# svenstaro/bvh

Hardware: NVIDIA H100
Metric: traversal_Mrays_per_s (higher is better)
Workload: dtype f32

## Files before the change

### bvh_b200/csrc/traverse.cu

```cuda
#include "internal.h"
#include "csr.cuh"
#include "queries.cuh"
#include <cstdlib>
#include <cstring>
#include <algorithm>
#include <chrono>

namespace bvhb200 {

static inline uint32_t pick_slots(bvhgpu_ctx* ctx, uint32_t nrays) {
    if (ctx->traverse_slots >= 0) return (uint32_t)std::min<int64_t>(ctx->traverse_slots, 64);
    uint64_t budget_words = 1ull << 30;
    if (ctx->slot_budget_words == 0) {
        size_t free_b = 0, total_b = 0;
        ctx->slot_budget_words = cudaMemGetInfo(&free_b, &total_b) == cudaSuccess ? std::max<uint64_t>((uint64_t)free_b / 16, 1) : budget_words;
    }
    budget_words = std::min<uint64_t>(budget_words, ctx->slot_budget_words);
    const uint64_t k = budget_words / std::max<uint32_t>(nrays, 1u);
    if (k < 4) return (uint32_t)k;
    uint32_t p = 4;
    while (p * 2 <= k && p < 64) p *= 2;
    return p;
}

template <class T> static inline const typename Traits<T>::DAabb* walk_aabbs(const Tree<T>* tree) { return tree->dims == 2 && tree->d_aabb_trav ? tree->d_aabb_trav : tree->d_aabb; }

constexpr int SCAN_ITEMS = 8;
constexpr int SCAN_THREADS = 256;
constexpr int SCAN_TILE = SCAN_ITEMS * SCAN_THREADS;
static_assert(SCAN_THREADS == CSR_SCAN_THREADS && SCAN_TILE == CSR_SCAN_TILE, "scan geometry declared in internal.h");

template <class T> __device__ __forceinline__ T tmin2(T a, T b);
template <> __device__ __forceinline__ float tmin2(float a, float b) { return fminf(a, b); }
template <> __device__ __forceinline__ double tmin2(double a, double b) { return fmin(a, b); }
template <class T> __device__ __forceinline__ T tmax2(T a, T b);
template <> __device__ __forceinline__ float tmax2(float a, float b) { return fmaxf(a, b); }
template <> __device__ __forceinline__ double tmax2(double a, double b) { return fmax(a, b); }

template <class T>
__device__ __forceinline__ bool slab_hit(const T o[3], const T inv[3], const T mn[3], const T mx[3]) {
    const T l0 = mul_rn(sub_rn(mn[0], o[0]), inv[0]), r0 = mul_rn(sub_rn(mx[0], o[0]), inv[0]);
    const T l1 = mul_rn(sub_rn(mn[1], o[1]), inv[1]), r1 = mul_rn(sub_rn(mx[1], o[1]), inv[1]);
    const T l2 = mul_rn(sub_rn(mn[2], o[2]), inv[2]), r2 = mul_rn(sub_rn(mx[2], o[2]), inv[2]);
    const bool nan = (l0 != l0) | (r0 != r0) | (l1 != l1) | (r1 != r1) | (l2 != l2) | (r2 != r2);
    const T tmin = tmax2(tmax2(tmin2(l0, r0), tmin2(l1, r1)), tmin2(l2, r2));
    const T tmax = tmin2(tmin2(tmax2(l0, r0), tmax2(l1, r1)), tmax2(l2, r2));
    const T lo = tmin > T(0) ? tmin : T(0);
    return !nan && tmax >= lo;
}
__device__ __forceinline__ float fmin_nan(float a, float b) { float r; asm("min.NaN.f32 %0, %1, %2;" : "=f"(r) : "f"(a), "f"(b)); return r; }
__device__ __forceinline__ float fmax_nan(float a, float b) { float r; asm("max.NaN.f32 %0, %1, %2;" : "=f"(r) : "f"(a), "f"(b)); return r; }
template <>
__device__ __forceinline__ bool slab_hit<float>(const float o[3], const float inv[3], const float mn[3], const float mx[3]) {
    const float l0 = mul_rn(sub_rn(mn[0], o[0]), inv[0]), r0 = mul_rn(sub_rn(mx[0], o[0]), inv[0]);
    const float l1 = mul_rn(sub_rn(mn[1], o[1]), inv[1]), r1 = mul_rn(sub_rn(mx[1], o[1]), inv[1]);
    const float l2 = mul_rn(sub_rn(mn[2], o[2]), inv[2]), r2 = mul_rn(sub_rn(mx[2], o[2]), inv[2]);
    const float tmin = fmax_nan(fmax_nan(fmin_nan(l0, r0), fmin_nan(l1, r1)), fmin_nan(l2, r2));
    const float tmax = fmin_nan(fmin_nan(fmax_nan(l0, r0), fmax_nan(l1, r1)), fmax_nan(l2, r2));
    const float lo = tmin > 0.f ? tmin : 0.f;
    return tmax >= lo;
}

template <class T, bool FLAT, class Emit>
__device__ __forceinline__ uint32_t walk(const typename Traits<T>::TNode* __restrict__ trec, uint32_t n_rec,
                                         const typename Traits<T>::DAabb* __restrict__ aabb,
                                         const T o[3], const T inv[3], Emit emit) {
    uint32_t i = 0, visits = 0;
    while (i < n_rec) {
        T mn[3], mx[3];
        uint32_t skip, shape;
        fetch(trec + i, mn, mx, skip, shape);
        ++visits;
        if (slab_hit(o, inv, mn, mx)) {
            if (shape != BVH_INVALID) {
                bool report = true;
                if (FLAT) {
                    T smn[3], smx[3];
                    load_aabb(aabb + shape, smn, smx);
                    report = slab_hit(o, inv, smn, smx);
                }
                if (report) emit(shape);
            }
            i = i + 1;
        } else {
            i = skip;
        }
    }
    return visits;
}

template <class T> struct RaySrc { const T* base; uint32_t fmt; };
constexpr uint32_t RAYS_FULL = 0, RAYS_OD = 1;
template <class T, bool L2>
__device__ __forceinline__ void load_ray(const RaySrc<T>& src, size_t r, T o[3], T inv[3]) {
    if (src.fmt == RAYS_FULL) {
        const T* p = src.base + 9 * r;
#pragma unroll
        for (int k = 0; k < 3; ++k) { o[k] = L2 ? __ldcg(p + k) : __ldg(p + k); inv[k] = L2 ? __ldcg(p + 6 + k) : __ldg(p + 6 + k); }
    } else {
        const T* p = src.base + 6 * r;
#pragma unroll
        for (int k = 0; k < 3; ++k) { o[k] = L2 ? __ldcg(p + k) : __ldg(p + k); inv[k] = div_rn(T(1), L2 ? __ldcg(p + 3 + k) : __ldg(p + 3 + k)); }
    }
}

template <class T>
__global__ void __launch_bounds__(256) coherence_probe_kernel(RaySrc<T> rays, uint32_t nrays, uint32_t* flag) {
    __shared__ float acc[8];
    float sum = 0.f;
    const uint32_t samples = 1024, stride = nrays > 2 * samples ? nrays / samples : 1;
    const uint32_t rstride = rays.fmt == RAYS_FULL ? 9u : 6u;
    uint32_t n = 0;
    for (uint32_t k = threadIdx.x; k < samples; k += 256) {
        const uint32_t i = k * stride;
        if (i + 1 >= nrays) break;
        const T* a = rays.base + (size_t)rstride * i + 3;
        const T* b = rays.base + (size_t)rstride * (i + 1) + 3;
        sum += (float)(a[0] * b[0] + a[1] * b[1] + a[2] * b[2]);
        ++n;
    }
    for (int o = 16; o > 0; o >>= 1) { sum += __shfl_xor_sync(0xffffffffu, sum, o); n += __shfl_xor_sync(0xffffffffu, n, o); }
    __shared__ uint32_t cnt[8];
    if (lane_id() == 0) { acc[threadIdx.x >> 5] = sum; cnt[threadIdx.x >> 5] = n; }
    __syncthreads();
    if (threadIdx.x == 0) {
        float s = 0.f; uint32_t c = 0;
        for (int w = 0; w < 8; ++w) { s += acc[w]; c += cnt[w]; }
        *flag = (c > 0 && s / (float)c > 0.9f) ? 1u : 0u;
    }
}

template <class T, bool FLAT>
__global__ void __launch_bounds__(256) walk_count_kernel(const typename Traits<T>::TNode* __restrict__ trec, uint32_t n_rec,
                                                         const typename Traits<T>::DAabb* __restrict__ aabb,
                                                         RaySrc<T> rays, uint32_t nrays,
                                                         uint32_t first, uint32_t count,
                                                         uint32_t* __restrict__ counts, uint32_t* __restrict__ slots, uint32_t K,
                                                         unsigned long long* __restrict__ visit_total, const uint32_t* __restrict__ gate, uint32_t run_if) {
    if (gate && *gate != run_if) return;
    const uint32_t r = first + blockIdx.x * blockDim.x + threadIdx.x;
    uint32_t visits = 0;
    if (r < first + count) {
        T o[3], inv[3];
        load_ray<T, false>(rays, r, o, inv);
        uint32_t cnt = 0;
        visits = walk<T, FLAT>(trec, n_rec, aabb, o, inv, [&](uint32_t shape) {
            if (cnt < K) slots[(size_t)cnt * nrays + r] = shape;
            ++cnt;
        });
        counts[r] = cnt;
    }
    visits = __reduce_add_sync(0xffffffffu, visits);
    if (lane_id() == 0 && visits) atomicAdd(visit_total, (unsigned long long)visits);
}

template <class T, bool FLAT, bool STREAM>
__global__ void __launch_bounds__(256) walk_persistent_kernel(const typename Traits<T>::TNode* __restrict__ trec, uint32_t n_rec,
                                                              const typename Traits<T>::DAabb* __restrict__ aabb,
                                                              RaySrc<T> rays, uint32_t nrays,
                                                              uint32_t* __restrict__ ticket, const uint32_t* ready,
                                                              uint32_t* __restrict__ counts, uint32_t* __restrict__ slots, uint32_t K,
                                                              unsigned long long* __restrict__ visit_total, const uint32_t* __restrict__ gate, uint32_t run_if,
                                                              uint32_t* err, unsigned long long timeout_ns) {
    if (gate && *gate != run_if) return;
    constexpr uint32_t NONE = 0xFFFFFFFFu;
    constexpr int REFILL = 8;
    const uint32_t FULL = 0xffffffffu;
    const uint32_t lane = lane_id(), lt = lanemask_lt();
    uint32_t r = NONE, i = 0, cnt = 0, visits = 0;
    bool loaded = false;
    T o[3] = {T(0), T(0), T(0)}, inv[3] = {T(0), T(0), T(0)};
    bool exhausted = false;
    for (;;) {
        const uint32_t need = __ballot_sync(FULL, r == NONE);
        if (need && !exhausted) {
            uint32_t base = 0;
            if (lane == 0) base = atomicAdd(ticket, (uint32_t)__popc(need));
            base = __shfl_sync(FULL, base, 0);
            if (base >= nrays) exhausted = true;
            const uint32_t mine = base + __popc(need & lt);
            if (r == NONE && mine < nrays) {
                r = mine; i = 0; cnt = 0;
                if (STREAM) loaded = false;
                else load_ray<T, false>(rays, mine, o, inv);
            }
        }
        if (STREAM) {
            const uint32_t pend = __ballot_sync(FULL, r != NONE && !loaded);
            if (pend) {
                const bool any_active = __ballot_sync(FULL, r != NONE && loaded) != 0u;
                const uint32_t lowest = __reduce_min_sync(FULL, (r != NONE && !loaded) ? r : NONE);
                uint32_t rd = 0, ok = 1;
                if (lane == 0) {
                    rd = *(volatile const uint32_t*)ready;
                    if (!any_active && rd <= lowest) {
                        uint32_t ns = 100;
                        const unsigned long long t0 = global_timer_ns();
                        while (rd <= lowest) {
                            if (*(volatile const uint32_t*)err != 0u) { ok = 0; break; }
                            if (global_timer_ns() - t0 > timeout_ns) { ok = 0; atomicExch(err, (uint32_t)BVHGPU_ERR_TIMEOUT); break; }
                            __nanosleep(ns);
                            if (ns < 2000) ns <<= 1;
                            rd = *(volatile const uint32_t*)ready;
                        }
                    }
                }
                rd = __shfl_sync(FULL, rd, 0);
                ok = __shfl_sync(FULL, ok, 0);
                if (!ok) {
                    exhausted = true;
                    if (r != NONE && !loaded) r = NONE;
                } else if (__ballot_sync(FULL, r != NONE && !loaded && r < rd)) {
                    __threadfence();
                    if (r != NONE && !loaded && r < rd) { load_ray<T, true>(rays, r, o, inv); loaded = true; }
                }
            }
        }
        if (__ballot_sync(FULL, r != NONE) == 0) break;
        uint32_t rounds = 0;
        for (;;) {
            if (r != NONE && (!STREAM || loaded)) {
                T mn[3], mx[3];
                uint32_t skip, shape;
                fetch(trec + i, mn, mx, skip, shape);
                ++visits;
                if (slab_hit(o, inv, mn, mx)) {
                    if (shape != BVH_INVALID) {
                        bool report = true;
                        if (FLAT) {
                            T smn[3], smx[3];
                            load_aabb(aabb + shape, smn, smx);
                            report = slab_hit(o, inv, smn, smx);
                        }
                        if (report) { if (cnt < K) slots[(size_t)cnt * nrays + r] = shape; ++cnt; }
                    }
                    i = i + 1;
                } else {
                    i = skip;
                }
                if (i >= n_rec) { counts[r] = cnt; r = NONE; }
            }
            const uint32_t idle_mask = __ballot_sync(FULL, r == NONE);
            const int idle = __popc(idle_mask);
            if (idle == 32 || (idle >= REFILL && !exhausted)) break;
            if (STREAM) {
                const uint32_t pend = __ballot_sync(FULL, r != NONE && !loaded);
                if (pend && (((++rounds) & 15u) == 0u || (pend | idle_mask) == FULL)) break;
            }
        }
    }
    visits = __reduce_add_sync(FULL, visits);
    if (lane == 0 && visits) atomicAdd(visit_total, (unsigned long long)visits);
}

template <bool FLAT, bool STREAM, int VPC>
__global__ void __launch_bounds__(1024, 1) walk_top_kernel(const TNodeF* __restrict__ trec, const DAabbF* __restrict__ aabb,
                                                           uint32_t n_rec, const float4* __restrict__ top,
                                                           RaySrc<float> rays, uint32_t nrays, uint32_t* __restrict__ ticket, const uint32_t* ready,
                                                           uint32_t* __restrict__ counts, uint32_t* __restrict__ slots, uint32_t K,
                                                           unsigned long long* __restrict__ visit_total, const uint32_t* __restrict__ gate, uint32_t run_if,
                                                           uint32_t* err, unsigned long long timeout_ns, int refill) {
    extern __shared__ float4 s_top[];
    if (gate && *gate != run_if) return;
    const uint32_t n_top = reinterpret_cast<const uint32_t*>(top)[0];
    for (uint32_t k = threadIdx.x; k < 2 * n_top; k += blockDim.x) s_top[k] = top[2 + k];
    __syncthreads();
    uint32_t s_lo, s_hi;
    asm volatile("mov.u32 %0, %1;" : "=r"(s_lo) : "r"((uint32_t)__cvta_generic_to_shared(s_top)));
    asm volatile("mov.u32 %0, %1;" : "=r"(s_hi) : "r"(s_lo + 16u * n_top));
    constexpr uint32_t NONE = 0xFFFFFFFFu;
    const uint32_t FULL = 0xffffffffu;
    const uint32_t lane = lane_id(), lt = lanemask_lt();
    uint32_t r = NONE, j = NONE, g = 0, gend = 0, cnt = 0, visits = 0;
    bool loaded = false;
    float o[3] = {0.f, 0.f, 0.f}, inv[3] = {0.f, 0.f, 0.f};
    float4 a = make_float4(0.f, 0.f, 0.f, 0.f), b = a;
    bool exhausted = false;
    for (;;) {
        const uint32_t need = __ballot_sync(FULL, r == NONE);
        if (need && !exhausted) {
            uint32_t base = 0;
            if (lane == 0) base = atomicAdd(ticket, (uint32_t)__popc(need));
            base = __shfl_sync(FULL, base, 0);
            if (base >= nrays) exhausted = true;
            const uint32_t mine = base + __popc(need & lt);
            if (r == NONE && mine < nrays) {
                r = mine; cnt = 0; g = 0;
                if (STREAM) { loaded = false; j = NONE; gend = 0; }
                else { j = 0; gend = n_top ? 0u : n_rec; load_ray<float, false>(rays, mine, o, inv); }
            }
        }
        if (STREAM) {
            const uint32_t pend = __ballot_sync(FULL, r != NONE && !loaded);
            if (pend) {
                const bool any_active = __ballot_sync(FULL, r != NONE && loaded) != 0u;
                const uint32_t lowest = __reduce_min_sync(FULL, (r != NONE && !loaded) ? r : NONE);
                uint32_t rd = 0, ok = 1;
                if (lane == 0) {
                    rd = *(volatile const uint32_t*)ready;
                    if (!any_active && rd <= lowest) {
                        uint32_t ns = 100;
                        const unsigned long long t0 = global_timer_ns();
                        while (rd <= lowest) {
                            if (*(volatile const uint32_t*)err != 0u) { ok = 0; break; }
                            if (global_timer_ns() - t0 > timeout_ns) { ok = 0; atomicExch(err, (uint32_t)BVHGPU_ERR_TIMEOUT); break; }
                            __nanosleep(ns);
                            if (ns < 2000) ns <<= 1;
                            rd = *(volatile const uint32_t*)ready;
                        }
                    }
                }
                rd = __shfl_sync(FULL, rd, 0);
                ok = __shfl_sync(FULL, ok, 0);
                if (!ok) {
                    exhausted = true;
                    if (r != NONE && !loaded) r = NONE;
                } else if (__ballot_sync(FULL, r != NONE && !loaded && r < rd)) {
                    __threadfence();
                    if (r != NONE && !loaded && r < rd) {
                        load_ray<float, true>(rays, r, o, inv); loaded = true;
                        j = 0; gend = n_top ? 0u : n_rec;
                    }
                }
            }
        }
        if (__ballot_sync(FULL, r != NONE) == 0) break;
        const int leave = exhausted ? 32 : refill;
        auto visit_branchy = [&]() {
            if (r != NONE && (!STREAM || loaded)) {
                float mn[3], mx[3];
                uint32_t w3, w7;
                const bool below = g < gend;
                if (!below) {
                    float4 lo4, hi4;
                    asm("ld.shared.v4.f32 {%0,%1,%2,%3}, [%4];" : "=f"(lo4.x), "=f"(lo4.y), "=f"(lo4.z), "=f"(lo4.w) : "r"(s_lo + 16u * j));
                    asm("ld.shared.v4.f32 {%0,%1,%2,%3}, [%4];" : "=f"(hi4.x), "=f"(hi4.y), "=f"(hi4.z), "=f"(hi4.w) : "r"(s_hi + 16u * j));
                    mn[0] = lo4.x; mn[1] = lo4.y; mn[2] = lo4.z; w3 = __float_as_uint(lo4.w);
                    mx[0] = hi4.x; mx[1] = hi4.y; mx[2] = hi4.z; w7 = __float_as_uint(hi4.w);
                } else {
                    fetch(trec + g, mn, mx, w3, w7);
                }
                ++visits;
                const bool hit = slab_hit(o, inv, mn, mx);
                const bool fringe = !below && (w7 + 0x80000000u) < 0x7FFFFFFFu;
                const uint32_t cur = below ? g : j;
                const uint32_t nxt = (hit || fringe) ? cur + 1 : w3;
                if (hit && (int32_t)w7 >= 0) {
                    bool report = true;
                    if (FLAT) {
// ... 88 lines not shown
    __shared__ unsigned long long wsum[32];
    __shared__ unsigned long long carry_s;
    if (threadIdx.x == 0) carry_s = *total;
    __syncthreads();
    for (uint32_t b0 = 0; b0 < nblocks; b0 += 1024) {
        const uint32_t b = b0 + threadIdx.x;
        const unsigned long long v = b < nblocks ? blocksum[b] : 0ull;
        unsigned long long incl = v;
#pragma unroll
        for (int o = 1; o < 32; o <<= 1) { const unsigned long long t = __shfl_up_sync(0xffffffffu, incl, o); if ((int)lane_id() >= o) incl += t; }
        if (lane_id() == 31) wsum[threadIdx.x >> 5] = incl;
        __syncthreads();
        unsigned long long woff = 0;
        for (int w = 0; w < (int)(threadIdx.x >> 5); ++w) woff += wsum[w];
        const unsigned long long carry = carry_s;
        if (b < nblocks) blocksum[b] = carry + woff + incl - v;
        __syncthreads();
        if (threadIdx.x == 1023) carry_s = carry + woff + incl;
        __syncthreads();
    }
    if (threadIdx.x == 0) *total = carry_s;
}

__device__ __forceinline__ void st_release_sys(unsigned long long* p, unsigned long long v) {
    asm volatile("st.release.sys.global.u64 [%0], %1;" ::"l"(p), "l"(v) : "memory");
}
__device__ __forceinline__ unsigned long long ld_acquire_sys(const unsigned long long* p) {
    unsigned long long v;
    asm volatile("ld.acquire.sys.global.u64 %0, [%1];" : "=l"(v) : "l"(p) : "memory");
    return v;
}
constexpr int MB_TOT = 0, MB_DONE = 64, MB_TRACE = 128, MB_TRACE_LEN = 1024;
constexpr unsigned long long TILE_BYTES = 4ull * SCAN_TILE;
constexpr unsigned long long OFF_MASK = (1ull << 56) - 1ull;
struct PeerBoxes {
    int rank, world;
    unsigned long long* box[BVHGPU_MAX_PEERS];
    unsigned char* stage[BVHGPU_MAX_PEERS];
    uint32_t* hits[BVHGPU_MAX_PEERS];
    unsigned long long seq;
    unsigned long long rays_before[BVHGPU_MAX_PEERS + 1];
    unsigned long long tiles_before[BVHGPU_MAX_PEERS + 1];
    unsigned long long table_off;
    uint32_t* err;
    unsigned long long timeout_ns;
};

struct XInfo { unsigned long long base[BVHGPU_MAX_PEERS], grand, waited; };
__device__ __forceinline__ void wait_posts(const PeerBoxes& pb, XInfo* xs) {
    const int lane = threadIdx.x;
    const unsigned long long par = pb.seq & 1ull;
    unsigned long long tot = 0, waited = 0;
    if (lane < pb.world) {
        const unsigned long long* slot = pb.box[pb.rank] + MB_TOT + (par * BVHGPU_MAX_PEERS + lane) * 4;
        const unsigned long long t0 = global_timer_ns();
        uint32_t spins = 0;
        while (ld_acquire_sys(slot) != pb.seq) {
            if (((++spins) & 63u) == 0u && global_timer_ns() - t0 > pb.timeout_ns) { atomicExch(pb.err, (uint32_t)BVHGPU_ERR_TIMEOUT); break; }
            __nanosleep(100);
        }
        tot = slot[1];
        waited = global_timer_ns() - t0;
    }
    unsigned long long run = 0, wmax = 0, mine = 0;
    for (int r = 0; r < pb.world; ++r) {
        const unsigned long long v = __shfl_sync(0xffffffffu, tot, r), w = __shfl_sync(0xffffffffu, waited, r);
        if (lane == r) mine = run;
        run += v;
        wmax = w > wmax ? w : wmax;
    }
    if (lane < BVHGPU_MAX_PEERS) xs->base[lane] = mine;
    if (lane == 0) { xs->grand = run; xs->waited = wmax; }
}

template <bool SHARDED>
__global__ void __launch_bounds__(SCAN_THREADS) scan_post_kernel(const uint32_t* __restrict__ counts, uint32_t n, uint32_t* __restrict__ local,
                                                                 unsigned long long* __restrict__ blocksum, unsigned long long* __restrict__ total,
                                                                 uint32_t* __restrict__ arrival, PeerBoxes pb, unsigned long long* __restrict__ xinfo) {
    __shared__ uint32_t wsum[SCAN_THREADS / 32], wmax[SCAN_THREADS / 32];
    __shared__ XInfo xs;
    __shared__ unsigned long long wsum64[SCAN_THREADS / 32];
    __shared__ unsigned long long carry_s;
    __shared__ bool last;
    const uint32_t base = blockIdx.x * SCAN_TILE + threadIdx.x * SCAN_ITEMS;
    uint32_t v[SCAN_ITEMS], s = 0, m = 0;
#pragma unroll
    for (int k = 0; k < SCAN_ITEMS; ++k) { v[k] = (base + k < n) ? counts[base + k] : 0u; s += v[k]; m = v[k] > m ? v[k] : m; }
    uint32_t incl = s;
#pragma unroll
    for (int o = 1; o < 32; o <<= 1) { const uint32_t t = __shfl_up_sync(0xffffffffu, incl, o); if ((int)lane_id() >= o) incl += t; }
    m = __reduce_max_sync(0xffffffffu, m);
    if (lane_id() == 31) wsum[threadIdx.x >> 5] = incl;
    if (lane_id() == 0) wmax[threadIdx.x >> 5] = m;
    __syncthreads();
    uint32_t woff = 0, tsum = 0, tmax = 0;
#pragma unroll
    for (int w = 0; w < SCAN_THREADS / 32; ++w) { if (w < (int)(threadIdx.x >> 5)) woff += wsum[w]; tsum += wsum[w]; tmax = wmax[w] > tmax ? wmax[w] : tmax; }
    uint32_t run = woff + incl - s;
#pragma unroll
    for (int k = 0; k < SCAN_ITEMS; ++k) { if (base + k < n) local[base + k] = run; run += v[k]; }
    const unsigned long long width = tmax <= 0xFFu ? 1ull : (tmax <= 0xFFFFu ? 2ull : 4ull);
    if (SHARDED) {
        unsigned long long tb_mine = 0;
#pragma unroll
        for (int k = 1; k < BVHGPU_MAX_PEERS; ++k) if (k == pb.rank) tb_mine = pb.tiles_before[k];
        const unsigned long long at = TILE_BYTES * (tb_mine + blockIdx.x) + (unsigned long long)threadIdx.x * SCAN_ITEMS * width;
        if (width == 1) {
            const uint2 q = make_uint2(v[0] | v[1] << 8 | v[2] << 16 | v[3] << 24, v[4] | v[5] << 8 | v[6] << 16 | v[7] << 24);
#pragma unroll
            for (int d = 0; d < BVHGPU_MAX_PEERS; ++d) if (d < pb.world) *reinterpret_cast<uint2*>(pb.stage[d] + at) = q;
        } else if (width == 2) {
            const uint4 q = make_uint4(v[0] | v[1] << 16, v[2] | v[3] << 16, v[4] | v[5] << 16, v[6] | v[7] << 16);
#pragma unroll
            for (int d = 0; d < BVHGPU_MAX_PEERS; ++d) if (d < pb.world) *reinterpret_cast<uint4*>(pb.stage[d] + at) = q;
        } else {
            const uint4 q0 = make_uint4(v[0], v[1], v[2], v[3]), q1 = make_uint4(v[4], v[5], v[6], v[7]);
#pragma unroll
            for (int d = 0; d < BVHGPU_MAX_PEERS; ++d) if (d < pb.world) { *reinterpret_cast<uint4*>(pb.stage[d] + at) = q0; *reinterpret_cast<uint4*>(pb.stage[d] + at + 16) = q1; }
        }
    }
    if (threadIdx.x == 0) blocksum[blockIdx.x] = (unsigned long long)tsum | (width << 56);
    __syncthreads();
    if (threadIdx.x == 0) {
        if (SHARDED && pb.world > 1) __threadfence_system(); else __threadfence();
        last = atomicAdd(arrival, 1u) == gridDim.x - 1;
    }
    __syncthreads();
    if (!last) return;
    if (threadIdx.x == 0) { __threadfence(); carry_s = 0ull; }
    __syncthreads();
    unsigned long long tb_mine = 0;
    if (SHARDED) {
#pragma unroll
        for (int k = 1; k < BVHGPU_MAX_PEERS; ++k) if (k == pb.rank) tb_mine = pb.tiles_before[k];
    }
    for (uint32_t b0 = 0; b0 < gridDim.x; b0 += SCAN_THREADS) {
        const uint32_t bb = b0 + threadIdx.x;
        const unsigned long long e = bb < gridDim.x ? __ldcg(blocksum + bb) : 0ull;
        const unsigned long long val = e & OFF_MASK;
        unsigned long long in64 = val;
#pragma unroll
        for (int o = 1; o < 32; o <<= 1) { const unsigned long long t = __shfl_up_sync(0xffffffffu, in64, o); if ((int)lane_id() >= o) in64 += t; }
        if (lane_id() == 31) wsum64[threadIdx.x >> 5] = in64;
        __syncthreads();
        unsigned long long wo = 0;
        for (int w = 0; w < (int)(threadIdx.x >> 5); ++w) wo += wsum64[w];
        const unsigned long long carry = carry_s;
        const unsigned long long excl = carry + wo + in64 - val;
        if (bb < gridDim.x) {
            blocksum[bb] = excl;
            if (SHARDED) {
                const unsigned long long entry = (excl & OFF_MASK) | (e & ~OFF_MASK);
#pragma unroll
                for (int d = 0; d < BVHGPU_MAX_PEERS; ++d) if (d < pb.world) *reinterpret_cast<unsigned long long*>(pb.stage[d] + pb.table_off + 8ull * (tb_mine + bb)) = entry;
            }
        }
        __syncthreads();
        if (threadIdx.x == SCAN_THREADS - 1) carry_s = carry + wo + in64;
        __syncthreads();
    }
    if (threadIdx.x == 0) { *total = carry_s; *arrival = 0u; }
    if (SHARDED) {
        if (threadIdx.x == 0) __threadfence_system();
        __syncthreads();
        if (threadIdx.x < (unsigned)pb.world) {
            unsigned long long* slot = pb.box[threadIdx.x] + MB_TOT + ((pb.seq & 1ull) * BVHGPU_MAX_PEERS + pb.rank) * 4;
// ... 123 lines not shown
    const uint32_t r = first + bid * blockDim.x + threadIdx.x;
    if (!sharded || failed == 0u) {
        if (r == first && dst.offsets) {
            const unsigned long long t = *total;
            dst.offsets[dst.nrays_out] = t > 0xFFFFFFFFull ? 0xFFFFFFFFu : (uint32_t)t;
        }
        if (r < first + count) {
            const unsigned long long off = hbase + blocksum[r / SCAN_TILE] + local[r];
            if (dst.offsets) dst.offsets[r] = off > 0xFFFFFFFFull ? 0xFFFFFFFFu : (uint32_t)off;
            const uint32_t c = counts[r];
            if (c != 0 && dst.hits != nullptr) {
                if (c <= K) {
                    for (uint32_t k0 = 0; k0 < c; k0 += 8) {
                        uint32_t h[8];
#pragma unroll
                        for (uint32_t j = 0; j < 8; ++j) if (k0 + j < c) h[j] = __ldcs(slots + (size_t)(k0 + j) * nrays + r);
#pragma unroll
                        for (uint32_t j = 0; j < 8; ++j) if (k0 + j < c && off + k0 + j < cap) dst.hits[off + k0 + j] = h[j];
                    }
                } else {
                    T o[3], inv[3];
                    load_ray<T, false>(rays, r, o, inv);
                    unsigned long long w = off;
                    walk<T, FLAT>(trec, n_rec, aabb, o, inv, [&](uint32_t shape) { if (w < cap) dst.hits[w] = shape; ++w; });
                }
            }
        }
    }
    if (!sharded) return;
    bool pushed = false;
    if (failed == 0u && pb.world > 1) {
        if (threadIdx.x == 0) {
            const uint32_t r0 = first + bid * blockDim.x;
            const uint32_t r1 = min(r0 + blockDim.x, first + count) - 1u;
            rng[0] = hbase + blocksum[r0 / SCAN_TILE] + local[r0];
            rng[1] = hbase + blocksum[r1 / SCAN_TILE] + local[r1] + counts[r1];
        }
        __syncthreads();
        const unsigned long long begin = rng[0], end = rng[1] < cap ? rng[1] : cap;
        if (begin < end) {
            pushed = true;
            const uint32_t* src = dst.hits;
            const unsigned long long q0 = (begin + 3ull) & ~3ull, q1 = end & ~3ull;
            if (q0 < q1) {
                for (unsigned long long q = (q0 >> 2) + threadIdx.x; q < (q1 >> 2); q += blockDim.x) {
                    const uint4 v = __ldcg(reinterpret_cast<const uint4*>(src) + q);
#pragma unroll
                    for (int d = 0; d < BVHGPU_MAX_PEERS; ++d) if (d < pb.world && d != pb.rank) reinterpret_cast<uint4*>(pb.hits[d])[q] = v;
                }
            }
            if (threadIdx.x < 8) {
                unsigned long long w;
                bool ok;
                if (q0 < q1) { w = threadIdx.x < 4 ? begin + threadIdx.x : q1 + (threadIdx.x - 4); ok = threadIdx.x < 4 ? w < q0 : w < end; }
                else         { w = begin + threadIdx.x; ok = w < end; }
                if (ok) {
                    const uint32_t v = __ldcg(src + w);
#pragma unroll
                    for (int d = 0; d < BVHGPU_MAX_PEERS; ++d) if (d < pb.world && d != pb.rank) pb.hits[d][w] = v;
                }
            }
        }
    }
    __syncthreads();
    if (threadIdx.x == 0) {
        if (pushed) __threadfence_system();
        last = atomicAdd(arrival, 1u) == nblocks - 1;
    }
    __syncthreads();
    if (!last) return;
    if (threadIdx.x == 0) { __threadfence_system(); *arrival = 0u; }
    __syncthreads();
    if (threadIdx.x < (unsigned)pb.world) st_release_sys(pb.box[threadIdx.x] + MB_DONE + (pb.seq & 1ull) * BVHGPU_MAX_PEERS + pb.rank, pb.seq);
}
template <class T, bool FLAT>
__global__ void __launch_bounds__(256) emit_kernel(const typename Traits<T>::TNode* __restrict__ trec, uint32_t n_rec,
                                                   const typename Traits<T>::DAabb* __restrict__ aabb,
                                                   RaySrc<T> rays, uint32_t nrays,
                                                   const uint32_t* __restrict__ counts, const uint32_t* __restrict__ slots, uint32_t K,
                                                   const uint32_t* __restrict__ local, const unsigned long long* __restrict__ blocksum,
                                                   const unsigned long long* __restrict__ total,
                                                   EmitDst dst, unsigned long long cap, uint32_t first, uint32_t count,
                                                   PeerBoxes pb, const unsigned long long* __restrict__ xinfo, uint32_t* __restrict__ arrival) {
    emit_body<T, FLAT>(trec, n_rec, aabb, rays, nrays, counts, slots, K, local, blocksum, total, dst, cap, first, count, pb, xinfo, arrival, blockIdx.x, gridDim.x);
}
template <class T, bool FLAT>
__global__ void __launch_bounds__(256) emit_goffsets_kernel(const typename Traits<T>::TNode* __restrict__ trec, uint32_t n_rec,
                                                            const typename Traits<T>::DAabb* __restrict__ aabb,
                                                            RaySrc<T> rays, uint32_t nrays,
                                                            const uint32_t* __restrict__ counts, const uint32_t* __restrict__ slots, uint32_t K,
                                                            const uint32_t* __restrict__ local, const unsigned long long* __restrict__ blocksum,
                                                            const unsigned long long* __restrict__ total,
                                                            EmitDst dst, unsigned long long cap, uint32_t count,
                                                            PeerBoxes pb, const unsigned long long* __restrict__ xinfo, uint32_t* __restrict__ arrival,
                                                            uint32_t emit_blocks, uint32_t* __restrict__ offsets) {
    if (blockIdx.x < emit_blocks) emit_body<T, FLAT>(trec, n_rec, aabb, rays, nrays, counts, slots, K, local, blocksum, total, dst, cap, 0u, count, pb, xinfo, arrival, blockIdx.x, emit_blocks);
    else goffsets_body(pb, xinfo, offsets, blockIdx.x - emit_blocks, gridDim.x - emit_blocks);
}

constexpr uint32_t SUMS_TAIL = 20;
constexpr uint32_t S_TOTAL = 0, S_VISITS = 1, S_XINFO = 2, S_ERR = 12, S_TICKET = 13, S_READY = 14, S_GATE = 15, S_MAXC = 16, S_BLKDONE = 17;
constexpr unsigned long long STREAM_TIMEOUT_NS = 4ull * 1000ull * 1000ull * 1000ull;
constexpr uint32_t TOP_BUDGET = 7000;
constexpr size_t TOP_UNROLL_MAX_BYTES = (size_t)32 << 20;
template <class T> static bool launch_top(Tree<T>*, bool, RaySrc<T>, uint32_t, uint32_t*, uint32_t*, uint32_t, unsigned long long*, uint32_t*, bool) { return false; }
template <> bool launch_top<float>(Tree<float>* tree, bool flat, RaySrc<float> rays, uint32_t R, uint32_t* counts, uint32_t* slots, uint32_t K,
                                   unsigned long long* tail, uint32_t* gate, bool stream_mode) {
    bvhgpu_ctx* ctx = tree->ctx;
    if (tree->n < 2) return false;
    const uint32_t budget = ctx->traverse_top > 1 ? (uint32_t)std::min<int64_t>(std::max<int64_t>(ctx->traverse_top, 8), TOP_BUDGET) : TOP_BUDGET;
    if ((!tree->top_valid || tree->top_budget != budget) && build_top_records(tree, budget) != BVHGPU_OK) return false;
    if (!ctx->top_attr_set) {
        const int bytes = (int)(TOP_BUDGET * 32);
        auto raise = [&](const void* f) { return cudaFuncSetAttribute(f, cudaFuncAttributeMaxDynamicSharedMemorySize, bytes) == cudaSuccess; };
        if (!raise((const void*)walk_top_kernel<false, false, 1>) || !raise((const void*)walk_top_kernel<true, false, 1>) ||
            !raise((const void*)walk_top_kernel<false, true, 1>) || !raise((const void*)walk_top_kernel<true, true, 1>) ||
            !raise((const void*)walk_top_kernel<false, false, 4>) || !raise((const void*)walk_top_kernel<true, false, 4>) ||
            !raise((const void*)walk_top_kernel<false, true, 4>) || !raise((const void*)walk_top_kernel<true, true, 4>)) { cudaGetLastError(); return false; }
        ctx->top_attr_set = true;
    }
    const size_t smem = (size_t)budget * 32;
    const int grid = (int)std::min<uint64_t>((uint64_t)ctx->sm_count, ((uint64_t)R + 1023) / 1024);
    uint32_t* ticket = reinterpret_cast<uint32_t*>(tail + S_TICKET);
    uint32_t* err = reinterpret_cast<uint32_t*>(tail + S_ERR);
    const float4* top = reinterpret_cast<const float4*>(tree->d_top);
    static const int top_refill = getenv("BVHGPU_TOP_REFILL") ? std::max(1, std::min(32, atoi(getenv("BVHGPU_TOP_REFILL")))) : 8;
    const bool l2_tree = (size_t)tree->n_trec * sizeof(TNodeF) <= TOP_UNROLL_MAX_BYTES;
#define BVH_TOP_LAUNCH(F, S, V, TMO) walk_top_kernel<F, S, V><<<grid, 1024, smem, ctx->stream>>>(tree->d_tnodes, walk_aabbs(tree), tree->n_trec, top, rays, R, ticket, \
                                                                    ctx->d_ready, counts, slots, K, tail + S_VISITS, gate, 0u, err, TMO, top_refill)
#define BVH_TOP_FORMS(V) do { if (stream_mode) { if (flat) BVH_TOP_LAUNCH(true, true, V, STREAM_TIMEOUT_NS); else BVH_TOP_LAUNCH(false, true, V, STREAM_TIMEOUT_NS); } \
                              else             { if (flat) BVH_TOP_LAUNCH(true, false, V, 0ull); else BVH_TOP_LAUNCH(false, false, V, 0ull); } } while (0)
    if (l2_tree) BVH_TOP_FORMS(4); else BVH_TOP_FORMS(1);
#undef BVH_TOP_FORMS
#undef BVH_TOP_LAUNCH
    ctx->launches++;
    return true;
}

template <class T>
static int launch_pass1(Tree<T>* tree, bool flat, RaySrc<T> rays, uint32_t R, uint32_t first, uint32_t count,
                        uint32_t* counts, uint32_t* slots, uint32_t K, unsigned long long* sums, uint32_t nblk, bool stream_mode) {
    bvhgpu_ctx* ctx = tree->ctx;
    cudaStream_t st = ctx->stream;
    unsigned long long* tail = sums + nblk;
    const int64_t pmode = stream_mode ? 1 : ctx->traverse_persistent;
    uint32_t* gate = nullptr;
    if (pmode >= 2) {
        gate = reinterpret_cast<uint32_t*>(tail + S_GATE);
        coherence_probe_kernel<T><<<1, 256, 0, st>>>(rays, R, gate);
        ctx->launches++;
    }
    if (pmode == 0 || pmode >= 2) {
        const int grid = (count + 255) / 256;
        if (flat) walk_count_kernel<T, true><<<grid, 256, 0, st>>>(tree->d_tnodes, tree->n_trec, walk_aabbs(tree), rays, R, first, count, counts, slots, K, tail + S_VISITS, gate, 1u);
        else      walk_count_kernel<T, false><<<grid, 256, 0, st>>>(tree->d_tnodes, tree->n_trec, walk_aabbs(tree), rays, R, first, count, counts, slots, K, tail + S_VISITS, gate, 1u);
        ctx->launches++;
        if (pmode == 0) return BVHGPU_OK;
    }
    if (first != 0 || count != R) { set_error("internal: persistent walk covers whole batches only"); return BVHGPU_ERR_INTERNAL; }
    const bool want_top = ctx->traverse_top >= 1 || (ctx->traverse_top < 0 && (size_t)tree->n_trec * sizeof(typename Traits<T>::TNode) >= ((size_t)5 << 20));
    if (want_top && launch_top(tree, flat, rays, R, counts, slots, K, tail, gate, stream_mode)) return BVHGPU_OK;
    if (ctx->walk_grid == 0) {
        int occ = 1;
        BVH_CUDA_TRY(cudaOccupancyMaxActiveBlocksPerMultiprocessor(&occ, walk_persistent_kernel<float, false, false>, 256, 0));
        ctx->walk_grid = ctx->sm_count * (occ < 1 ? 1 : occ);
    }
    const uint64_t sms = (uint64_t)ctx->sm_count;
    const uint64_t per_sm = std::min<uint64_t>((uint64_t)ctx->walk_grid / sms, std::max<uint64_t>(4, (uint64_t)R / (6ull * 256ull * sms)));
    const int grid = (int)std::min<uint64_t>(ctx->walk_grid_forced ? (uint64_t)ctx->walk_grid : std::max<uint64_t>(1, per_sm) * sms, ((uint64_t)R + 255) / 256);
    uint32_t* ticket = reinterpret_cast<uint32_t*>(tail + S_TICKET);
    const uint32_t* ready = ctx->d_ready;
    uint32_t* err = reinterpret_cast<uint32_t*>(tail + S_ERR);
    if (stream_mode) {
        if (flat) walk_persistent_kernel<T, true, true><<<grid, 256, 0, st>>>(tree->d_tnodes, tree->n_trec, walk_aabbs(tree), rays, R, ticket, ready, counts, slots, K, tail + S_VISITS, nullptr, 0u, err, STREAM_TIMEOUT_NS);
        else      walk_persistent_kernel<T, false, true><<<grid, 256, 0, st>>>(tree->d_tnodes, tree->n_trec, walk_aabbs(tree), rays, R, ticket, ready, counts, slots, K, tail + S_VISITS, nullptr, 0u, err, STREAM_TIMEOUT_NS);
    } else {
        if (flat) walk_persistent_kernel<T, true, false><<<grid, 256, 0, st>>>(tree->d_tnodes, tree->n_trec, walk_aabbs(tree), rays, R, ticket, ready, counts, slots, K, tail + S_VISITS, gate, 0u, err, 0ull);
        else      walk_persistent_kernel<T, false, false><<<grid, 256, 0, st>>>(tree->d_tnodes, tree->n_trec, walk_aabbs(tree), rays, R, ticket, ready, counts, slots, K, tail + S_VISITS, gate, 0u, err, 0ull);
    }
    ctx->launches++;
    return BVHGPU_OK;
}

template <class T>
int traverse_device(Tree<T>* tree, int mode, const void* d_rays, uint32_t fmt, size_t nrays,
                    uint32_t* d_offsets, uint32_t* d_hits, size_t cap, size_t* total, const bvhgpu_shard* shard) {
    bvhgpu_ctx* ctx = tree->ctx;
    cudaStream_t st = ctx->stream;
    if (nrays > 0x7FFFFFFFull) { set_error("traverse: nrays %zu exceeds 2^31-1", nrays); return BVHGPU_ERR_INVALID; }
    if (mode != BVHGPU_TRAVERSE_BVH && mode != BVHGPU_TRAVERSE_FLAT) { set_error("traverse: bad mode %d", mode); return BVHGPU_ERR_INVALID; }
    if (fmt != RAYS_FULL && fmt != RAYS_OD) { set_error("traverse: bad ray layout %u", fmt); return BVHGPU_ERR_INVALID; }
    tree->last_nrays = nrays;
    if (nrays == 0) {
        if (d_offsets) BVH_CUDA_TRY(cudaMemsetAsync(d_offsets, 0, sizeof(uint32_t), st));
        if (total) *total = 0;
        tree->last_total = 0;
        return BVHGPU_OK;
    }
    if (tree->n == 0) {
        BVH_CUDA_TRY(cudaMemsetAsync(d_offsets, 0, sizeof(uint32_t) * (nrays + 1), st));
        if (total) *total = 0;
        tree->last_total = 0;
        return BVHGPU_OK;
    }
    BVH_TRY(resolve_status(tree));
    if (!tree->d_tnodes) BVH_TRY(build_traversal_records(tree));
    const RaySrc<T> rays{reinterpret_cast<const T*>(d_rays), fmt};
    const uint32_t R = (uint32_t)nrays;
    const uint32_t K = pick_slots(ctx, R);
    const uint32_t nblk = (R + SCAN_TILE - 1) / SCAN_TILE;
    Scratch scratch(ctx);
    uint32_t *counts = nullptr, *slots = nullptr, *local = nullptr;
    unsigned long long* sums = nullptr;
    BVH_TRY(scratch.get(&counts, R));
    BVH_TRY(scratch.get(&local, R));
    if (K) BVH_TRY(scratch.get(&slots, (size_t)K * R));
    BVH_TRY(scratch.get(&sums, (size_t)nblk + SUMS_TAIL));
    unsigned long long* tail = sums + nblk;
    BVH_CUDA_TRY(cudaMemsetAsync(tail, 0, SUMS_TAIL * sizeof(unsigned long long), st));
    const bool flat = mode == BVHGPU_TRAVERSE_FLAT;
    {
        if (ctx->profile) cudaEventRecord(ctx->ev_walk[0], st);
        BVH_TRY(launch_pass1<T>(tree, flat, rays, R, 0, R, counts, slots, K, sums, nblk, false));
        if (ctx->profile) { cudaEventRecord(ctx->ev_walk[1], st); ctx->have_walk = true; }
    }
    const int grid = (R + 255) / 256;
    EmitDst dst{};
    PeerBoxes pb{};
    uint32_t* arrival = reinterpret_cast<uint32_t*>(tail + S_BLKDONE);
    if (shard) {
        const int W = shard->world;
        pb.rank = shard->rank; pb.world = W; pb.seq = shard->seq;
        pb.err = ctx->d_async_err; pb.timeout_ns = 10ull * 1000ull * 1000ull * 1000ull;
        pb.rays_before[0] = 0; pb.tiles_before[0] = 0;
        for (int d = 0; d < BVHGPU_MAX_PEERS; ++d) {
            const unsigned long long nd = d < W ? (unsigned long long)shard->shard_rays[d] : 0ull;
            pb.rays_before[d + 1] = pb.rays_before[d] + nd;
            pb.tiles_before[d + 1] = pb.tiles_before[d] + (nd + SCAN_TILE - 1) / SCAN_TILE;
        }
        const unsigned long long NG = pb.rays_before[W], NT = pb.tiles_before[W];
        pb.table_off = TILE_BYTES * NT;
        const size_t half = BVHGPU_SHARD_STAGE_BYTES(NG);
        if (pb.table_off + 8ull * NT > half) { set_error("internal: staging layout exceeds BVHGPU_SHARD_STAGE_BYTES"); return BVHGPU_ERR_INTERNAL; }
        for (int d = 0; d < W; ++d) {
            pb.box[d] = (unsigned long long*)shard->peer_mailbox[d];
            pb.stage[d] = (unsigned char*)shard->peer_counts[d] + (shard->seq & 1ull) * half;
            pb.hits[d] = (uint32_t*)shard->peer_hits[d];
        }
        if (shard->shard_rays[shard->rank] != nrays) { set_error("traverse_sharded: shard_rays[rank] = %zu but nrays = %zu", shard->shard_rays[shard->rank], nrays); return BVHGPU_ERR_INVALID; }
        if (NG > 0x7FFFFFFFull) { set_error("traverse_sharded: %llu rays in total exceed 2^31-1", NG); return BVHGPU_ERR_INVALID; }
        cap = shard->cap;
        dst.offsets = nullptr; dst.hits = pb.hits[pb.rank];
        scan_post_kernel<true><<<nblk, SCAN_THREADS, 0, st>>>(counts, R, local, sums, tail + S_TOTAL, arrival, pb, tail + S_XINFO);
    } else {
        dst.offsets = d_offsets; dst.hits = d_hits; dst.nrays_out = R;
        scan_post_kernel<false><<<nblk, SCAN_THREADS, 0, st>>>(counts, R, local, sums, tail + S_TOTAL, arrival, pb, tail + S_XINFO);
    }
    ctx->launches++;
    unsigned long long* h = reinterpret_cast<unsigned long long*>(ctx->h_pinned);
    if (total) {
        BVH_CUDA_TRY(cudaMemcpyAsync(h, tail, 2 * sizeof(unsigned long long), cudaMemcpyDeviceToHost, st));
        BVH_CUDA_TRY(cudaEventRecord(ctx->ev_total, st));
    }
    if (shard) {
        const unsigned g2 = (unsigned)grid + (unsigned)pb.tiles_before[pb.world];
        if (flat) emit_goffsets_kernel<T, true><<<g2, 256, 0, st>>>(tree->d_tnodes, tree->n_trec, walk_aabbs(tree), rays, R, counts, slots, K, local, sums, tail + S_TOTAL, dst, (unsigned long long)cap, R, pb, tail + S_XINFO, arrival, (uint32_t)grid, (uint32_t*)shard->offsets);
        else      emit_goffsets_kernel<T, false><<<g2, 256, 0, st>>>(tree->d_tnodes, tree->n_trec, walk_aabbs(tree), rays, R, counts, slots, K, local, sums, tail + S_TOTAL, dst, (unsigned long long)cap, R, pb, tail + S_XINFO, arrival, (uint32_t)grid, (uint32_t*)shard->offsets);
    } else {
        if (flat) emit_kernel<T, true><<<grid, 256, 0, st>>>(tree->d_tnodes, tree->n_trec, walk_aabbs(tree), rays, R, counts, slots, K, local, sums, tail + S_TOTAL, dst, (unsigned long long)cap, 0u, R, pb, tail + S_XINFO, arrival);
        else      emit_kernel<T, false><<<grid, 256, 0, st>>>(tree->d_tnodes, tree->n_trec, walk_aabbs(tree), rays, R, counts, slots, K, local, sums, tail + S_TOTAL, dst, (unsigned long long)cap, 0u, R, pb, tail + S_XINFO, arrival);
    }
    ctx->launches++;
    BVH_CUDA_TRY(cudaGetLastError());
    int rc = BVHGPU_OK;
    if (total) {
        BVH_CUDA_TRY(cudaEventSynchronize(ctx->ev_total));
        *total = (size_t)h[0];
        tree->last_total = (size_t)h[0];
        tree->last_visits = h[1];
        if (h[0] > 0xFFFFFFFFull) { set_error("traverse: %llu hits overflow the u32 CSR offsets", h[0]); rc = BVHGPU_ERR_CAPACITY; }
        else if (d_hits && h[0] > cap) { set_error("traverse: %llu hits do not fit capacity %zu", h[0], cap); rc = BVHGPU_ERR_CAPACITY; }
    }
    return rc;
}

__global__ void overlap_probe_kernel(const volatile uint32_t* flag, uint32_t* saw, unsigned long long timeout_ns) {
    const unsigned long long t0 = global_timer_ns();
    uint32_t ok = 0;
    for (;;) {
        if (*flag) { ok = 1; break; }
        if (global_timer_ns() - t0 > timeout_ns) break;
        __nanosleep(200);
    }
    *saw = ok;
}
static bool tooling_detected() {
    const char* lb = getenv("CUDA_LAUNCH_BLOCKING");
    if (lb && lb[0] && strcmp(lb, "0") != 0) return true;
    static const char* vars[] = {"CUDA_INJECTION64_PATH", "CUDA_INJECTION32_PATH", "NV_CUDA_START_SUSPENDED", "NVIDIA_PROCESS_INJECTION_CRASH_REPORTING",
                                 "NVIDIA_PROCESS_INJECTION_XML_TARGET_SETTINGS", "CUDBG_USE_LEGACY_DEBUGGER", "NV_NSIGHT_INJECTION_TRANSPORT_TYPE",
                                 "NSIGHT_CUDA_DEBUGGER", "CUDA_DEBUGGER_SOFTWARE_PREEMPTION"};
    for (const char* v : vars) { const char* e = getenv(v); if (e && e[0]) return true; }
    static int mapped = -1;
    if (mapped < 0) {
        int found = 0;
        if (FILE* f = fopen("/proc/self/maps", "r")) {
            char line[1024];
            while (!found && fgets(line, sizeof line, f))
                if (strstr(line, "nsight") || strstr(line, "libcuda-injection") || strstr(line, "libsanitizer-collection") || strstr(line, "libInterceptorInjection") || strstr(line, "libTreeLauncher"))
                    found = 1;
            fclose(f);
        }
        mapped = found;
    }
    return mapped == 1;
}
static int stream_capable(bvhgpu_ctx* ctx) {
    if (ctx->traverse_stream == 0) return 0;
    if (ctx->traverse_stream == 1) return 1;
    if (tooling_detected()) return 0;
    if (ctx->stream_ok >= 0) return ctx->stream_ok;
    ctx->stream_ok = 0;
    uint32_t* d = nullptr;
    if (dalloc_t(ctx, &d, 2) != BVHGPU_OK) return 0;
    uint32_t* h = ctx->h_pinned + 128;
    bool ok = cudaMemsetAsync(d, 0, 2 * sizeof(uint32_t), ctx->stream) == cudaSuccess;
    ok = ok && cudaEventRecord(ctx->ev_order, ctx->stream) == cudaSuccess && cudaStreamWaitEvent(ctx->copy_stream, ctx->ev_order, 0) == cudaSuccess;
    if (ok) {
        overlap_probe_kernel<<<1, 1, 0, ctx->stream>>>(d, d + 1, 20ull * 1000ull * 1000ull);
        h[0] = 1u;
        ok = cudaMemcpyAsync(d, h, sizeof(uint32_t), cudaMemcpyHostToDevice, ctx->copy_stream) == cudaSuccess;
        ok = ok && cudaMemcpyAsync(h + 1, d + 1, sizeof(uint32_t), cudaMemcpyDeviceToHost, ctx->stream) == cudaSuccess;
        ok = (cudaStreamSynchronize(ctx->copy_stream) == cudaSuccess) && ok;
        ok = (cudaStreamSynchronize(ctx->stream) == cudaSuccess) && ok;
        ctx->launches++;
        if (ok && h[1] == 1u) ctx->stream_ok = 1;
    }
    dfree(ctx, d);
    return ctx->stream_ok;
}

typedef int (*WriteValue32Fn)(cudaStream_t, unsigned long long, uint32_t, unsigned int);
static WriteValue32Fn stream_write_value32() {
    static WriteValue32Fn fn = nullptr;
    static bool tried = false;
    if (!tried) {
        tried = true;
        void* p = nullptr;
        cudaDriverEntryPointQueryResult q;
        if (cudaGetDriverEntryPoint("cuStreamWriteValue32", &p, cudaEnableDefault, &q) == cudaSuccess && q == cudaDriverEntryPointSuccess) fn = (WriteValue32Fn)p;
        else (void)cudaGetLastError();
    }
    return fn;
// ... 424 lines not shown
```

Baseline: 2675.

## Use programmatic dependent launch to overlap probe, walk, scan and emit kernels

Adds griddepcontrol wait/launch_dependents to the probe, walk, top-walk, scan and emit kernels, and launches them via cudaLaunchKernelEx with programmatic stream serialization so each kernel's prologue can overlap the previous kernel's tail. The top-level walk now loads its shared-memory top tree before waiting on the gated probe. The gated count kernel is reordered to launch after the persistent kernel. The probe kernel also batches its sample loads so they can be issued together. The aim is to hide launch latency and inter-kernel gaps, at the cost of more complex ordering that could introduce races if a wait is misplaced.

```diff
diff --git a/bvh_b200/csrc/traverse.cu b/bvh_b200/csrc/traverse.cu
--- a/bvh_b200/csrc/traverse.cu
+++ b/bvh_b200/csrc/traverse.cu
@@ -104,19 +104,31 @@
     }
 }
 
+__device__ __forceinline__ void wait_prior_grid() { asm volatile("griddepcontrol.wait;" ::: "memory"); }
+__device__ __forceinline__ void allow_next_grid() { asm volatile("griddepcontrol.launch_dependents;" ::: "memory"); }
+
 template <class T>
 __global__ void __launch_bounds__(256) coherence_probe_kernel(RaySrc<T> rays, uint32_t nrays, uint32_t* flag) {
     __shared__ float acc[8];
+    allow_next_grid();
     float sum = 0.f;
-    const uint32_t samples = 1024, stride = nrays > 2 * samples ? nrays / samples : 1;
+    constexpr uint32_t samples = 1024, per_thread = samples / 256;
+    const uint32_t stride = nrays > 2 * samples ? nrays / samples : 1;
     const uint32_t rstride = rays.fmt == RAYS_FULL ? 9u : 6u;
     uint32_t n = 0;
-    for (uint32_t k = threadIdx.x; k < samples; k += 256) {
-        const uint32_t i = k * stride;
-        if (i + 1 >= nrays) break;
-        const T* a = rays.base + (size_t)rstride * i + 3;
-        const T* b = rays.base + (size_t)rstride * (i + 1) + 3;
-        sum += (float)(a[0] * b[0] + a[1] * b[1] + a[2] * b[2]);
+    T a[per_thread][3], b[per_thread][3];
+#pragma unroll
+    for (uint32_t q = 0; q < per_thread; ++q) {
+        const uint32_t i = (threadIdx.x + 256 * q) * stride;
+        if (i + 1 < nrays) {
+#pragma unroll
+            for (int c = 0; c < 3; ++c) { a[q][c] = rays.base[(size_t)rstride * i + 3 + c]; b[q][c] = rays.base[(size_t)rstride * (i + 1) + 3 + c]; }
+        }
+    }
+#pragma unroll
+    for (uint32_t q = 0; q < per_thread; ++q) {
+        if ((threadIdx.x + 256 * q) * stride + 1 >= nrays) break;
+        sum += (float)(a[q][0] * b[q][0] + a[q][1] * b[q][1] + a[q][2] * b[q][2]);
         ++n;
     }
     for (int o = 16; o > 0; o >>= 1) { sum += __shfl_xor_sync(0xffffffffu, sum, o); n += __shfl_xor_sync(0xffffffffu, n, o); }
@@ -137,6 +149,8 @@
                                                          uint32_t first, uint32_t count,
                                                          uint32_t* __restrict__ counts, uint32_t* __restrict__ slots, uint32_t K,
                                                          unsigned long long* __restrict__ visit_total, const uint32_t* __restrict__ gate, uint32_t run_if) {
+    allow_next_grid();
+    wait_prior_grid();
     if (gate && *gate != run_if) return;
     const uint32_t r = first + blockIdx.x * blockDim.x + threadIdx.x;
     uint32_t visits = 0;
@@ -261,10 +275,11 @@
                                                            unsigned long long* __restrict__ visit_total, const uint32_t* __restrict__ gate, uint32_t run_if,
                                                            uint32_t* err, unsigned long long timeout_ns, int refill) {
     extern __shared__ float4 s_top[];
-    if (gate && *gate != run_if) return;
     const uint32_t n_top = reinterpret_cast<const uint32_t*>(top)[0];
     for (uint32_t k = threadIdx.x; k < 2 * n_top; k += blockDim.x) s_top[k] = top[2 + k];
     __syncthreads();
+    wait_prior_grid();
+    if (gate && *gate != run_if) return;
     uint32_t s_lo, s_hi;
     asm volatile("mov.u32 %0, %1;" : "=r"(s_lo) : "r"((uint32_t)__cvta_generic_to_shared(s_top)));
     asm volatile("mov.u32 %0, %1;" : "=r"(s_hi) : "r"(s_lo + 16u * n_top));
@@ -519,6 +534,8 @@
     __shared__ unsigned long long wsum64[SCAN_THREADS / 32];
     __shared__ unsigned long long carry_s;
     __shared__ bool last;
+    wait_prior_grid();
+    allow_next_grid();
     const uint32_t base = blockIdx.x * SCAN_TILE + threadIdx.x * SCAN_ITEMS;
     uint32_t v[SCAN_ITEMS], s = 0, m = 0;
 #pragma unroll
@@ -808,6 +825,7 @@
                                                    const unsigned long long* __restrict__ total,
                                                    EmitDst dst, unsigned long long cap, uint32_t first, uint32_t count,
                                                    PeerBoxes pb, const unsigned long long* __restrict__ xinfo, uint32_t* __restrict__ arrival) {
+    wait_prior_grid();
     emit_body<T, FLAT>(trec, n_rec, aabb, rays, nrays, counts, slots, K, local, blocksum, total, dst, cap, first, count, pb, xinfo, arrival, blockIdx.x, gridDim.x);
 }
 template <class T, bool FLAT>
@@ -824,18 +842,31 @@
     else goffsets_body(pb, xinfo, offsets, blockIdx.x - emit_blocks, gridDim.x - emit_blocks);
 }
 
+template <class... P, class... A>
+static cudaError_t launch_kernel(void (*kernel)(P...), unsigned grid, unsigned block, size_t smem, cudaStream_t st, bool pdl, A&&... args) {
+    cudaLaunchAttribute attr{};
+    attr.id = cudaLaunchAttributeProgrammaticStreamSerialization;
+    attr.val.programmaticStreamSerializationAllowed = 1;
+    cudaLaunchConfig_t cfg{};
+    cfg.gridDim = dim3(grid); cfg.blockDim = dim3(block); cfg.dynamicSmemBytes = smem; cfg.stream = st;
+    cfg.attrs = &attr; cfg.numAttrs = pdl ? 1 : 0;
+    return cudaLaunchKernelEx(&cfg, kernel, std::forward<A>(args)...);
+}
+
 constexpr uint32_t SUMS_TAIL = 20;
 constexpr uint32_t S_TOTAL = 0, S_VISITS = 1, S_XINFO = 2, S_ERR = 12, S_TICKET = 13, S_READY = 14, S_GATE = 15, S_MAXC = 16, S_BLKDONE = 17;
 constexpr unsigned long long STREAM_TIMEOUT_NS = 4ull * 1000ull * 1000ull * 1000ull;
 constexpr uint32_t TOP_BUDGET = 7000;
 constexpr size_t TOP_UNROLL_MAX_BYTES = (size_t)32 << 20;
-template <class T> static bool launch_top(Tree<T>*, bool, RaySrc<T>, uint32_t, uint32_t*, uint32_t*, uint32_t, unsigned long long*, uint32_t*, bool) { return false; }
+template <class T> static bool launch_top(Tree<T>*, bool, RaySrc<T>, uint32_t, uint32_t*, uint32_t*, uint32_t, unsigned long long*, uint32_t*, bool, bool) { return false; }
 template <> bool launch_top<float>(Tree<float>* tree, bool flat, RaySrc<float> rays, uint32_t R, uint32_t* counts, uint32_t* slots, uint32_t K,
-                                   unsigned long long* tail, uint32_t* gate, bool stream_mode) {
+                                   unsigned long long* tail, uint32_t* gate, bool stream_mode, bool after_probe) {
     bvhgpu_ctx* ctx = tree->ctx;
     if (tree->n < 2) return false;
     const uint32_t budget = ctx->traverse_top > 1 ? (uint32_t)std::min<int64_t>(std::max<int64_t>(ctx->traverse_top, 8), TOP_BUDGET) : TOP_BUDGET;
-    if ((!tree->top_valid || tree->top_budget != budget) && build_top_records(tree, budget) != BVHGPU_OK) return false;
+    const bool rebuild = !tree->top_valid || tree->top_budget != budget;
+    if (rebuild && build_top_records(tree, budget) != BVHGPU_OK) return false;
+    const bool pdl = after_probe && !rebuild;
     if (!ctx->top_attr_set) {
         const int bytes = (int)(TOP_BUDGET * 32);
         auto raise = [&](const void* f) { return cudaFuncSetAttribute(f, cudaFuncAttributeMaxDynamicSharedMemorySize, bytes) == cudaSuccess; };
@@ -852,8 +883,8 @@
     const float4* top = reinterpret_cast<const float4*>(tree->d_top);
     static const int top_refill = getenv("BVHGPU_TOP_REFILL") ? std::max(1, std::min(32, atoi(getenv("BVHGPU_TOP_REFILL")))) : 8;
     const bool l2_tree = (size_t)tree->n_trec * sizeof(TNodeF) <= TOP_UNROLL_MAX_BYTES;
-#define BVH_TOP_LAUNCH(F, S, V, TMO) walk_top_kernel<F, S, V><<<grid, 1024, smem, ctx->stream>>>(tree->d_tnodes, walk_aabbs(tree), tree->n_trec, top, rays, R, ticket, \
-                                                                    ctx->d_ready, counts, slots, K, tail + S_VISITS, gate, 0u, err, TMO, top_refill)
+#define BVH_TOP_LAUNCH(F, S, V, TMO) launch_kernel(walk_top_kernel<F, S, V>, grid, 1024, smem, ctx->stream, pdl, tree->d_tnodes, walk_aabbs(tree), tree->n_trec, top, rays, R, \
+                                                  ticket, ctx->d_ready, counts, slots, K, tail + S_VISITS, gate, 0u, err, TMO, top_refill)
 #define BVH_TOP_FORMS(V) do { if (stream_mode) { if (flat) BVH_TOP_LAUNCH(true, true, V, STREAM_TIMEOUT_NS); else BVH_TOP_LAUNCH(false, true, V, STREAM_TIMEOUT_NS); } \
                               else             { if (flat) BVH_TOP_LAUNCH(true, false, V, 0ull); else BVH_TOP_LAUNCH(false, false, V, 0ull); } } while (0)
     if (l2_tree) BVH_TOP_FORMS(4); else BVH_TOP_FORMS(1);
@@ -870,22 +901,24 @@
     cudaStream_t st = ctx->stream;
     unsigned long long* tail = sums + nblk;
     const int64_t pmode = stream_mode ? 1 : ctx->traverse_persistent;
-    uint32_t* gate = nullptr;
-    if (pmode >= 2) {
-        gate = reinterpret_cast<uint32_t*>(tail + S_GATE);
+    uint32_t* gate = pmode >= 2 ? reinterpret_cast<uint32_t*>(tail + S_GATE) : nullptr;
+    auto launch_count = [&](bool pdl) -> int {
+        const unsigned grid = (count + 255) / 256;
+        if (!pdl && flat) walk_count_kernel<T, true><<<grid, 256, 0, st>>>(tree->d_tnodes, tree->n_trec, walk_aabbs(tree), rays, R, first, count, counts, slots, K, tail + S_VISITS, gate, 1u);
+        else if (!pdl)    walk_count_kernel<T, false><<<grid, 256, 0, st>>>(tree->d_tnodes, tree->n_trec, walk_aabbs(tree), rays, R, first, count, counts, slots, K, tail + S_VISITS, gate, 1u);
+        else BVH_CUDA_TRY(launch_kernel(flat ? walk_count_kernel<T, true> : walk_count_kernel<T, false>, grid, 256, 0, st, true,
+                                        tree->d_tnodes, tree->n_trec, walk_aabbs(tree), rays, R, first, count, counts, slots, K, tail + S_VISITS, gate, 1u));
+        ctx->launches++;
+        return BVHGPU_OK;
+    };
+    if (pmode == 0) return launch_count(false);
+    if (gate) {
         coherence_probe_kernel<T><<<1, 256, 0, st>>>(rays, R, gate);
         ctx->launches++;
     }
-    if (pmode == 0 || pmode >= 2) {
-        const int grid = (count + 255) / 256;
-        if (flat) walk_count_kernel<T, true><<<grid, 256, 0, st>>>(tree->d_tnodes, tree->n_trec, walk_aabbs(tree), rays, R, first, count, counts, slots, K, tail + S_VISITS, gate, 1u);
-        else      walk_count_kernel<T, false><<<grid, 256, 0, st>>>(tree->d_tnodes, tree->n_trec, walk_aabbs(tree), rays, R, first, count, counts, slots, K, tail + S_VISITS, gate, 1u);
-        ctx->launches++;
-        if (pmode == 0) return BVHGPU_OK;
-    }
     if (first != 0 || count != R) { set_error("internal: persistent walk covers whole batches only"); return BVHGPU_ERR_INTERNAL; }
     const bool want_top = ctx->traverse_top >= 1 || (ctx->traverse_top < 0 && (size_t)tree->n_trec * sizeof(typename Traits<T>::TNode) >= ((size_t)5 << 20));
-    if (want_top && launch_top(tree, flat, rays, R, counts, slots, K, tail, gate, stream_mode)) return BVHGPU_OK;
+    if (want_top && launch_top(tree, flat, rays, R, counts, slots, K, tail, gate, stream_mode, gate != nullptr)) return gate ? launch_count(true) : BVHGPU_OK;
     if (ctx->walk_grid == 0) {
         int occ = 1;
         BVH_CUDA_TRY(cudaOccupancyMaxActiveBlocksPerMultiprocessor(&occ, walk_persistent_kernel<float, false, false>, 256, 0));
@@ -905,7 +938,7 @@
         else      walk_persistent_kernel<T, false, false><<<grid, 256, 0, st>>>(tree->d_tnodes, tree->n_trec, walk_aabbs(tree), rays, R, ticket, ready, counts, slots, K, tail + S_VISITS, gate, 0u, err, 0ull);
     }
     ctx->launches++;
-    return BVHGPU_OK;
+    return gate ? launch_count(true) : BVHGPU_OK;
 }
 
 template <class T>
@@ -980,7 +1013,7 @@
         scan_post_kernel<true><<<nblk, SCAN_THREADS, 0, st>>>(counts, R, local, sums, tail + S_TOTAL, arrival, pb, tail + S_XINFO);
     } else {
         dst.offsets = d_offsets; dst.hits = d_hits; dst.nrays_out = R;
-        scan_post_kernel<false><<<nblk, SCAN_THREADS, 0, st>>>(counts, R, local, sums, tail + S_TOTAL, arrival, pb, tail + S_XINFO);
+        BVH_CUDA_TRY(launch_kernel(scan_post_kernel<false>, nblk, SCAN_THREADS, 0, st, !ctx->profile, counts, R, local, sums, tail + S_TOTAL, arrival, pb, tail + S_XINFO));
     }
     ctx->launches++;
     unsigned long long* h = reinterpret_cast<unsigned long long*>(ctx->h_pinned);
@@ -993,8 +1026,9 @@
         if (flat) emit_goffsets_kernel<T, true><<<g2, 256, 0, st>>>(tree->d_tnodes, tree->n_trec, walk_aabbs(tree), rays, R, counts, slots, K, local, sums, tail + S_TOTAL, dst, (unsigned long long)cap, R, pb, tail + S_XINFO, arrival, (uint32_t)grid, (uint32_t*)shard->offsets);
         else      emit_goffsets_kernel<T, false><<<g2, 256, 0, st>>>(tree->d_tnodes, tree->n_trec, walk_aabbs(tree), rays, R, counts, slots, K, local, sums, tail + S_TOTAL, dst, (unsigned long long)cap, R, pb, tail + S_XINFO, arrival, (uint32_t)grid, (uint32_t*)shard->offsets);
     } else {
-        if (flat) emit_kernel<T, true><<<grid, 256, 0, st>>>(tree->d_tnodes, tree->n_trec, walk_aabbs(tree), rays, R, counts, slots, K, local, sums, tail + S_TOTAL, dst, (unsigned long long)cap, 0u, R, pb, tail + S_XINFO, arrival);
-        else      emit_kernel<T, false><<<grid, 256, 0, st>>>(tree->d_tnodes, tree->n_trec, walk_aabbs(tree), rays, R, counts, slots, K, local, sums, tail + S_TOTAL, dst, (unsigned long long)cap, 0u, R, pb, tail + S_XINFO, arrival);
+        const bool pdl = total == nullptr;
+        BVH_CUDA_TRY(launch_kernel(flat ? emit_kernel<T, true> : emit_kernel<T, false>, grid, 256, 0, st, pdl, tree->d_tnodes, tree->n_trec, walk_aabbs(tree), rays, R,
+                                   counts, slots, K, local, sums, tail + S_TOTAL, dst, (unsigned long long)cap, 0u, R, pb, tail + S_XINFO, arrival));
     }
     ctx->launches++;
     BVH_CUDA_TRY(cudaGetLastError());
```

Measured after the change: 2717, median of 6. 1.02x the previous value.
